# martenlienen/generative-turbulence

Hardware: AMD Instinct MI355X
Metric: U-Net fwd+bwd voxels/sec (DDPM training step, 192x64x48x4) (higher is better)
Workload: dtype bf16

## Files before the change

generative-turbulence_amd/csrc/tdx_conv3_ring.hip:

```cpp
#include "tdx_common.h"
#include "tdx_conv3.h"
#include "tdx_mfma.h"
#include <stdlib.h>
#include <algorithm>

#define RG_HY 10
#define RG_SZ 12
#define RG_SZ4 6
#define RG_WSLOTS 3
#define RG_WAVES 8
#define RG_STEPS 14
#ifndef RG_DEFAULT_LOADERS
#define RG_DEFAULT_LOADERS 1
#endif

struct RingArgs {
    const bf16* x1; const bf16* x2; int C1, C2;
    const bf16* wp; const float* bias; bf16* y;
    int B, X, Y, Z, Cout;
    int nbx, nby, nbz, ntn;
    double* gn_acc;
    bf16* d1; bf16* d2; int D1; const bf16* a1; const bf16* a2;
    const void* zeros;
    unsigned long long* stamps;
};

__device__ __forceinline__ void rg_dma_off(const void* sbase, unsigned voff, unsigned lds) {
    lds = __builtin_amdgcn_readfirstlane(lds);
    unsigned keep;
    asm volatile("s_mov_b32 %0, m0\n\ts_mov_b32 m0, %3\n\ts_nop 0\n\tglobal_load_lds_dwordx4 %1, %2\n\ts_mov_b32 m0, %0"
                 : "=&s"(keep) : "v"(voff), "s"(sbase), "s"(lds) : "memory");
}
#define RG_VMCNT(n) asm volatile("s_waitcnt vmcnt(%0)" ::"n"(n) : "memory")

#ifdef RG_STAMPS
#define RG_NSTAMP 64
#define RG_T()                                                                                        \
    do {                                                                                              \
        if (ord >= RG_STAMP_B0 && ord < RG_STAMP_B0 + 2) {                                            \
            const unsigned long long t_ = __builtin_amdgcn_s_memtime();                               \
            if (lane == 0 && nst < RG_NSTAMP) sStamp[wave * RG_NSTAMP + nst] = t_;                    \
            ++nst;                                                                                    \
        }                                                                                             \
    } while (0)
#else
#define RG_T() do { } while (0)
#endif

template <int BN>
__device__ __forceinline__ int rg_tile_addr(int v, int c) {
    if (BN == 64) return v * 128 + ((c ^ (v & 7)) << 4);
    return v * 64 + ((c ^ ((v >> 1) & 3)) << 4);
}

template <int NT, int LW = 0, bool Z4 = false>
struct RingShape {
    static constexpr int IW = LW ? LW : 8;
    static constexpr int BN = NT * 32;
    static constexpr int MT = 4 / NT;
    static constexpr int XP = Z4 ? MT : MT / 2;
    static constexpr int BX = 8 * XP;
    static constexpr int BZ = Z4 ? 4 : 8;
    static constexpr int HZ = BZ + 2;
    static constexpr int SZ = Z4 ? RG_SZ4 : RG_SZ;
    static constexpr int ENT = Z4 ? (BX + 2) / 2 * RG_HY * RG_SZ
                                  : (BX + 2) * RG_HY * SZ;
    static constexpr int APIECES = (ENT + 63) / 64;
    static constexpr int ABUF = APIECES * 1024;
    static constexpr int BPW = (APIECES + IW - 1) / IW;
    static constexpr int WPIECES = 28 * BN * 16 / 1024;
    static constexpr int WSLOT = WPIECES * 1024;
    static constexpr int WPW = (WPIECES + IW - 1) / IW;
    static constexpr int TILE = 32 * BN * 2;
    static constexpr int CH = BN / 8;
    static constexpr int VPI = 64 / CH;
    static constexpr int NST = MT * (32 / VPI);
    static constexpr size_t LDS = (size_t)2 * ABUF + (size_t)RG_WSLOTS * WSLOT + (size_t)RG_WAVES * TILE + 1024  +
                                  64  + BN * 4  + (size_t)RG_WAVES * BN * 2 * 4 ;
};

template <int NT, bool ZP, int LW, bool HF, bool Z4>
__global__ void __launch_bounds__(512 + 64 * LW, LW ? 3 : 2) conv3_ring_kernel(RingArgs A) {
    typedef RingShape<NT, LW, Z4> S;
    typedef H16<HF> H;
    typedef typename H::T HT;
    constexpr int BN = S::BN, MT = S::MT, XP = S::XP, BPW = S::BPW, WPW = S::WPW, CH = S::CH, VPI = S::VPI, NST = S::NST;
    static_assert(LW > 0 || BPW + WPW < RG_STEPS, "one DMA instruction per K step");
    extern __shared__ __attribute__((aligned(1024))) unsigned char smem[];
    unsigned char* sA = smem;
    unsigned char* sW = sA + 2 * S::ABUF;
    unsigned char* sT = sW + RG_WSLOTS * S::WSLOT;
    unsigned char* sD = sT + RG_WAVES * S::TILE;
    unsigned char* sZ = sD + 1024;
    float* sBias = reinterpret_cast<float*>(sZ + 64);
    float* sRed = sBias + BN;
    const unsigned lds0 = (unsigned)(size_t)(__attribute__((address_space(3))) const void*)smem;
    const unsigned ldsA = lds0, ldsW = lds0 + 2 * S::ABUF, ldsD = ldsW + RG_WSLOTS * S::WSLOT + RG_WAVES * S::TILE;

    const int tid = threadIdx.x, lane = tid & 63;
    const int wave = __builtin_amdgcn_readfirstlane(tid >> 6);
    const int r = lane & 31, hh = lane >> 5;
    const bool loader = LW > 0 && wave >= RG_WAVES;
    const int iw = LW ? wave - RG_WAVES : wave;
#ifdef RG_STAMPS
    unsigned long long* sStamp = reinterpret_cast<unsigned long long*>(NT == 2 ? sRed : sRed + RG_WAVES * BN * 2);
    int nst = 0;
#endif

    const int hw = blockIdx.x, xcd = hw & 7, slot = hw >> 3;
    const int ntile = slot % A.ntn, kx = slot / A.ntn, KX = (int)(gridDim.x >> 3) / A.ntn;
    const int nbricks = A.B * A.nbx * A.nby * A.nbz;
    const int lo = xcd * (nbricks >> 3) + min(xcd, nbricks & 7), hi = lo + (nbricks >> 3) + (xcd < (nbricks & 7) ? 1 : 0);
    const int nmine = hi - lo > kx ? (hi - lo - kx + KX - 1) / KX : 0;
    if (nmine == 0) return;
    const int n0 = ntile * BN;
    const int Cin = A.C1 + A.C2, nun = Cin >> 3;
    const int YZ = A.Y * A.Z, V = A.X * YZ;

    if (tid < BN) sBias[tid] = A.bias ? A.bias[n0 + tid] : 0.f;
    if (tid < 16) reinterpret_cast<unsigned*>(sZ)[tid] = 0u;
    lds_barrier();

    int hxyz[BPW];
#pragma unroll
    for (int i = 0; i < BPW; ++i) {
        const int pi = min(max(iw, 0) * BPW + i, S::APIECES - 1);
        const int e = min(pi * 64 + lane, S::ENT - 1);
        int hx, hy, hz;
        if (Z4) {
            const int xp = e / (RG_HY * RG_SZ), rem = e - xp * (RG_HY * RG_SZ), q = rem % RG_SZ;
            hy = rem / RG_SZ; hx = 2 * xp + q / RG_SZ4; hz = q % RG_SZ4;
        } else {
            hx = e / (RG_HY * S::SZ);
            const int rem = e - hx * (RG_HY * S::SZ);
            hy = rem / S::SZ; hz = min(rem - hy * S::SZ, S::HZ - 1);
        }
        hxyz[i] = hx | (hy << 8) | (hz << 16);
    }
    unsigned wlane[WPW];
#pragma unroll
    for (int j = 0; j < WPW; ++j) {
        const int pj = min(max(iw, 0) * WPW + j, S::WPIECES - 1);
        const int e = pj * 64 + lane;
        wlane[j] = (unsigned)((min(e / BN, 26) * A.Cout + (e % BN)) * 32);
    }

    const int ly = Z4 ? (r & 7) : (r & 3), lz = Z4 ? (r >> 3) : (r >> 2);
    int a_h[MT];
#pragma unroll
    for (int mt = 0; mt < MT; ++mt) {
        const int px = Z4 ? wave * XP + mt : wave * XP + mt / 2, py = Z4 ? ly : 4 * (mt % 2) + ly;
        const int hx = px + 1;
        a_h[mt] = Z4 ? ((hx >> 1) * (RG_HY * RG_SZ) + (py + 1) * RG_SZ + (hx & 1) * RG_SZ4 + (lz + 1)) * 16
                     : ((hx * RG_HY + (py + 1)) * S::SZ + (lz + 1)) * 16;
    }
    int xo[Z4 ? 2 : 1][RG_STEPS];
#pragma unroll
    for (int p = 0; p < RG_STEPS; ++p) {
        const int t = min(2 * p + hh, 26);
        const int dx = t / 9 - 1, dy = (t / 3) % 3 - 1, dz = t % 3 - 1;
        if (Z4) {
            const int step_odd = dx > 0 ? RG_HY * RG_SZ - RG_SZ4 : (dx < 0 ? -RG_SZ4 : 0);
            const int step_even = dx > 0 ? RG_SZ4 : (dx < 0 ? RG_SZ4 - RG_HY * RG_SZ : 0);
            xo[0][p] = (step_odd + dy * RG_SZ + dz) * 16;
            xo[Z4 ? 1 : 0][p] = (step_even + dy * RG_SZ + dz) * 16;
        } else {
            xo[0][p] = ((dx * RG_HY + dy) * S::SZ + dz) * 16;
        }
    }
    int b_off[NT];
#pragma unroll
    for (int nt = 0; nt < NT; ++nt) b_off[nt] = (hh * BN + nt * 32 + r) * 16;

    int vox[BPW];
    int vb_b = 0;
    auto brick_coords = [&](int ord, int& b, int& o0, int& o1, int& o2) {
        int id = lo + kx + KX * ord;
        const int bz = id % A.nbz; id /= A.nbz;
        const int by = id % A.nby; id /= A.nby;
        const int bx = id % A.nbx; id /= A.nbx;
        b = id; o0 = bx * S::BX; o1 = by * 8; o2 = bz * S::BZ;
    };
    auto plan_brick = [&](int ord) {
        int b, o0, o1, o2;
        brick_coords(min(ord, nmine - 1), b, o0, o1, o2);
        vb_b = b;
#pragma unroll
        for (int i = 0; i < BPW; ++i) {
            int s0 = o0 + (hxyz[i] & 0xff) - 1, s1 = o1 + ((hxyz[i] >> 8) & 0xff) - 1, s2 = o2 + ((hxyz[i] >> 16) & 0xff) - 1;
            bool ok = true;
            if (ZP) ok = s0 >= 0 && s0 < A.X && s1 >= 0 && s1 < A.Y && s2 >= 0 && s2 < A.Z;
            else { s0 = min(max(s0, 0), A.X - 1); s1 = min(max(s1, 0), A.Y - 1); s2 = min(max(s2, 0), A.Z - 1); }
            vox[i] = ok ? (s0 * A.Y + s1) * A.Z + s2 : -1;
        }
    };
    auto issue_brick_piece = [&](int c8, int buf, int i) {
        const int k0 = c8 << 3;
        const bf16* xs; int Cs, kk;
        if (k0 < A.C1) { xs = A.x1; Cs = A.C1; kk = k0; } else { xs = A.x2; Cs = A.C2; kk = k0 - A.C1; }
        const bf16* base = xs + ((int64_t)vb_b * V) * Cs + kk;
        const int pi = iw * BPW + i;
        const unsigned dst = pi < S::APIECES ? ldsA + buf * S::ABUF + pi * 1024 : ldsD;
        if (ZP) {
            const bf16* src = vox[i] >= 0 ? base + (int64_t)vox[i] * Cs : reinterpret_cast<const bf16*>(A.zeros);
            lds_dma16(src, dst);
        } else {
            rg_dma_off(base, (unsigned)(vox[i] * Cs) * 2u, dst);
        }
    };
    auto issue_weight_piece = [&](int c8, int wslot, int j) {
        const bf16* base = A.wp + ((int64_t)((c8 >> 1) * 27) * A.Cout + n0) * 16 + (c8 & 1) * 8;
        const int pj = iw * WPW + j;
        const unsigned dst = pj < S::WPIECES ? ldsW + wslot * S::WSLOT + pj * 1024 : ldsD;
        rg_dma_off(base, wlane[j], dst);
    };

    typedef __attribute__((ext_vector_type(2))) float f32x2;
    f32x2 p1[4], p2[4];
#pragma unroll
    for (int e = 0; e < 4; ++e) p1[e] = p2[e] = f32x2{0.f, 0.f};
    auto flush_stats = [&](int b) {
        float s1[8], s2[8];
#pragma unroll
        for (int e = 0; e < 4; ++e) { s1[2 * e] = p1[e].x; s1[2 * e + 1] = p1[e].y; s2[2 * e] = p2[e].x; s2[2 * e + 1] = p2[e].y; }
#pragma unroll
        for (int e = 0; e < 8; ++e) {
#pragma unroll
            for (int o = CH; o < 64; o <<= 1) { s1[e] += __shfl_xor(s1[e], o, 64); s2[e] += __shfl_xor(s2[e], o, 64); }
        }
        if (lane < CH) {
#pragma unroll
            for (int e = 0; e < 8; ++e) {
                sRed[(wave * BN + lane * 8 + e) * 2] = s1[e];
                sRed[(wave * BN + lane * 8 + e) * 2 + 1] = s2[e];
            }
        }
        lds_barrier();
        if (tid < BN * 2) {
            float t = 0.f;
#pragma unroll
            for (int w = 0; w < RG_WAVES; ++w) t += sRed[w * BN * 2 + tid];
            const int rep = blockIdx.x & (TDX_GN_REPLICAS - 1);
            atomicAdd(&A.gn_acc[(((size_t)rep * A.B + b) * A.Cout + n0) * 2 + tid], (double)t);
        }
        lds_barrier();
#pragma unroll
        for (int e = 0; e < 4; ++e) p1[e] = p2[e] = f32x2{0.f, 0.f};
    };

    int qs = 1, qb = 0, ws = 2 % nun, uw = 2;
    int u = 0;
    if (LW == 0 || loader) {
        plan_brick(0);
#pragma unroll
        for (int i = 0; i < BPW; ++i) issue_brick_piece(0, 0, i);
#pragma unroll
        for (int j = 0; j < WPW; ++j) issue_weight_piece(0, 0, j);
#pragma unroll
        for (int j = 0; j < WPW; ++j) issue_weight_piece(1 % nun, 1, j);
        if (qs == nun) { qs = 0; qb = 1; plan_brick(1); }
    }
    if (LW > 0 && loader) {
        for (int ord = 0; ord < nmine; ++ord) {
            for (int c8 = 0; c8 < nun; ++c8, ++u) {
                RG_VMCNT(WPW);
                lds_barrier();
#pragma unroll
                for (int i = 0; i < BPW; ++i) issue_brick_piece(qs, (u + 1) & 1, i);
#pragma unroll
                for (int j = 0; j < WPW; ++j) issue_weight_piece(ws, uw % RG_WSLOTS, j);
                ++uw;
                if (++ws == nun) ws = 0;
                if (++qs == nun) { qs = 0; ++qb; plan_brick(qb); }
            }
#ifndef RG_STAMPS
            if (!ZP && A.gn_acc != nullptr) {
                int b, nb = -1, t0, t1, t2;
                brick_coords(ord, b, t0, t1, t2);
                if (ord + 1 < nmine) brick_coords(ord + 1, nb, t0, t1, t2);
                if (nb != b) { lds_barrier(); lds_barrier(); }
            }
#endif
        }
        RG_VMCNT(0);
        return;
    }
    bool stores_behind = false;

    f32x16 acc[NT][MT];

    for (int ord = 0; ord < nmine; ++ord) {
        int b, o0, o1, o2;
        brick_coords(ord, b, o0, o1, o2);
#pragma unroll
        for (int nt = 0; nt < NT; ++nt)
#pragma unroll
            for (int j = 0; j < 4; ++j) {
                const float4 bv = *reinterpret_cast<const float4*>(sBias + nt * 32 + 8 * j + 4 * hh);
#pragma unroll
                for (int mt = 0; mt < MT; ++mt) {
                    acc[nt][mt][4 * j] = bv.x; acc[nt][mt][4 * j + 1] = bv.y; acc[nt][mt][4 * j + 2] = bv.z; acc[nt][mt][4 * j + 3] = bv.w;
                }
            }

        for (int c8 = 0; c8 < nun; ++c8, ++u) {
            RG_T();
            if (LW == 0) { if (stores_behind) RG_VMCNT(WPW + NST); else RG_VMCNT(WPW); }
            stores_behind = false;
            RG_T();
            lds_barrier();
            RG_T();

            const unsigned char* bufA = sA + (u & 1) * S::ABUF;
            const unsigned char* slotW = sW + (u % RG_WSLOTS) * S::WSLOT;
            const unsigned char* xa[MT];
#pragma unroll
            for (int mt = 0; mt < MT; ++mt) xa[mt] = bufA + a_h[mt];

            bf16x8 xf[3][MT], wf[3][NT];
            auto read_frags = [&](int p, int fb) {
#pragma unroll
                for (int mt = 0; mt < MT; ++mt) {
                    const unsigned char* src = xa[mt] + xo[Z4 ? (mt & 1) : 0][p];
                    if (p == RG_STEPS - 1) src = hh ? sZ : src;
                    xf[fb][mt] = *reinterpret_cast<const bf16x8*>(src);
                }
#pragma unroll
                for (int nt = 0; nt < NT; ++nt) wf[fb][nt] = *reinterpret_cast<const bf16x8*>(slotW + p * (2 * BN * 16) + b_off[nt]);
            };
            read_frags(0, 0);
            read_frags(1, 1);
            __builtin_amdgcn_sched_group_barrier(0x100, 2 * (MT + NT), 0);
#pragma unroll
            for (int p = 0; p < RG_STEPS; ++p) {
#if defined(RG_ABL) && (RG_ABL & 2)
                if (false)
#endif
                if (p + 2 < RG_STEPS) read_frags(p + 2, (p + 2) % 3);
#pragma unroll
                for (int nt = 0; nt < NT; ++nt)
#pragma unroll
                    for (int mt = 0; mt < MT; ++mt)
                        acc[nt][mt] = H::mfma(wf[p % 3][nt], xf[p % 3][mt], acc[nt][mt]);
                if (p + 2 < RG_STEPS) {
#pragma unroll
                    for (int k = 0; k < 4; ++k) {
                        __builtin_amdgcn_sched_group_barrier(0x008, 1, 0);
                        if (k < MT + NT) __builtin_amdgcn_sched_group_barrier(0x100, 1, 0);
                    }
                } else {
                    __builtin_amdgcn_sched_group_barrier(0x008, 4, 0);
                }
#if !defined(RG_ABL) || !(RG_ABL & 1)
                if (LW == 0 && p < BPW) issue_brick_piece(qs, (u + 1) & 1, p);
                if (LW == 0 && p >= BPW && p < BPW + WPW) issue_weight_piece(ws, uw % RG_WSLOTS, p - BPW);
#endif
                if (LW == 0 && p == BPW + WPW) {
                    ++uw;
                    if (++ws == nun) ws = 0;
                    if (++qs == nun) { qs = 0; ++qb; plan_brick(qb); }
                }
            }
        }

        RG_T();
        unsigned char* tile = sT + wave * S::TILE;
        const int last_b = b;
#pragma unroll
        for (int mt = 0; mt < MT; ++mt) {
            const int vw = ly * S::BZ + lz;
#pragma unroll
            for (int nt = 0; nt < NT; ++nt)
#pragma unroll
                for (int j = 0; j < 4; ++j) {
                    const int ch = nt * 32 + 8 * j + 4 * hh;
                    const unsigned lo2 = H::pack2(acc[nt][mt][4 * j], acc[nt][mt][4 * j + 1]);
                    const unsigned hi2 = H::pack2(acc[nt][mt][4 * j + 2], acc[nt][mt][4 * j + 3]);
                    *reinterpret_cast<uint2*>(tile + rg_tile_addr<BN>(vw, ch >> 3) + (ch & 7) * 2) = make_uint2(lo2, hi2);
                }
#pragma unroll
            for (int i = 0; i < 32 / VPI; ++i) {
                const int v = lane / CH + VPI * i, cidx = lane % CH;
                const int c0 = o0 + (Z4 ? wave * XP + mt : wave * XP + mt / 2);
                const int c1 = o1 + (Z4 ? (v >> 2) : 4 * (mt % 2) + (v >> 3)), c2 = o2 + (Z4 ? (v & 3) : (v & 7));
                uint4 val = *reinterpret_cast<const uint4*>(tile + rg_tile_addr<BN>(v, cidx));
                const int64_t ov = (int64_t)b * V + c0 * YZ + c1 * A.Z + c2;
                const int n = n0 + cidx * 8;
                if (ZP) {
                    const bool lo1 = n < A.D1;
                    bf16* dst = lo1 ? A.d1 + ov * A.D1 + n : A.d2 + ov * (A.Cout - A.D1) + (n - A.D1);
                    const bf16* asrc = lo1 ? (A.a1 ? A.a1 + ov * A.D1 + n : nullptr)
                                           : (A.a2 ? A.a2 + ov * (A.Cout - A.D1) + (n - A.D1) : nullptr);
                    if (asrc) {
                        Vec8<HT> va, vb;
                        va.load(reinterpret_cast<const HT*>(&val));
                        vb.load(reinterpret_cast<const HT*>(asrc));
#pragma unroll
                        for (int e = 0; e < 8; ++e) va.v[e] += vb.v[e];
                        va.store(reinterpret_cast<HT*>(dst));
                    } else {
                        *reinterpret_cast<uint4*>(dst) = val;
                    }
                } else {
                    *reinterpret_cast<uint4*>(A.y + ov * A.Cout + n) = val;
                    if (A.gn_acc != nullptr) {
                        const unsigned wds[4] = {val.x, val.y, val.z, val.w};
#pragma unroll
                        for (int e = 0; e < 4; ++e) {
                            const f32x2 lh = {H::lo(wds[e]), H::hi(wds[e])};
                            p1[e] += lh;
                            p2[e] = __builtin_elementwise_fma(lh, lh, p2[e]);
                        }
                    }
                }
            }
        }
        stores_behind = true;
        RG_T();
#ifndef RG_STAMPS
        if (!ZP && A.gn_acc != nullptr) {
            int nb = -1;
            if (ord + 1 < nmine) { int t0, t1, t2; brick_coords(ord + 1, nb, t0, t1, t2); }
            if (nb != last_b) flush_stats(last_b);
        }
#endif
    }
    if (LW == 0) RG_VMCNT(0);
#ifdef RG_STAMPS
    if (lane == 0 && A.stamps != nullptr) {
        unsigned long long* rec = A.stamps + ((size_t)blockIdx.x * RG_WAVES + wave) * (RG_NSTAMP + 1);
        rec[0] = nst;
        for (int i = 0; i < RG_NSTAMP; ++i) rec[1 + i] = sStamp[wave * RG_NSTAMP + i];
    }
#endif
}

static bool ring_z8_supported(int C1, int C2, int Cout, int B, int X, int Y, int Z, int mode);
static bool ring_z4_supported(int C1, int C2, int Cout, int B, int X, int Y, int Z, int mode) {
    const char* env = getenv("TDX_RING_Z4");
    if (env && atoi(env) == 0) return false;
    const int NT = Cout % 64 == 0 ? 2 : 1, bx = NT == 2 ? 16 : 32;
    if (X < bx || Y < 8 || Z < 4 || (X % bx) > 2 || (Y % 8) > 2 || (Z % 4) > 2) return false;
    const int ntn = Cout / (32 * NT);
    if (ntn > tdx_persistent_cus() / 8) return false;
    if ((int64_t)X * Y * Z * 1024 >= (1ll << 31)) return false;
    if (mode == 2) return true;
    if (NT == 1 && std::max(C1, C2) > 32) return false;
    const int64_t nb = (int64_t)B * (X / bx) * (Y / 8) * (Z / 4);
    return nb * ntn >= 192 && (C1 + C2) >= 64;
}
static int ring_brick_depth(int C1, int C2, int Cout, int B, int X, int Y, int Z) {
    const char* env = getenv("TDX_CONV3_RING");
    const int mode = env ? atoi(env) : 1;
    if (mode == 0 || !conv3_mfma_supported(C1, C2, Cout)) return 0;
    const char* z4 = getenv("TDX_RING_Z4");
    if (z4 && atoi(z4) == 2 && ring_z4_supported(C1, C2, Cout, B, X, Y, Z, 2)) return 4;
    if (ring_z8_supported(C1, C2, Cout, B, X, Y, Z, mode)) return 8;
    return ring_z4_supported(C1, C2, Cout, B, X, Y, Z, mode) ? 4 : 0;
}
int conv3_ring_depth(int C1, int C2, int N, int B, int X, int Y, int Z, bool data_gradient) {
    if (data_gradient && (tdx_scratch_ptr() == nullptr || tdx_scratch_bytes() < 16)) return 0;
    return ring_brick_depth(C1, C2, N, B, X, Y, Z);
}
static bool ring_z8_supported(int C1, int C2, int Cout, int B, int X, int Y, int Z, int mode) {
    const int NT = Cout % 64 == 0 ? 2 : 1, bx = NT == 2 ? 8 : 16;
    if (X < bx || Y < 8 || Z < 8 || (X % bx) > 2 || (Y % 8) > 2 || (Z % 8) > 2) return false;
    const char* rag = getenv("TDX_RING_RAGGED");
    if (rag && atoi(rag) == 0 && ((X % bx) || (Y % 8) || (Z % 8))) return false;
    const int ntn = Cout / (32 * NT);
    if (ntn > tdx_persistent_cus() / 8) return false;
    if ((int64_t)X * Y * Z * 1024 >= (1ll << 31)) return false;
    if (mode == 2) return true;
    if (NT == 1 && std::max(C1, C2) > 32) return false;
    const int64_t nb = (int64_t)B * (X / bx) * (Y / 8) * (Z / 8);
    const char* mi = getenv("TDX_RING_MIN_ITEMS");
    return nb * ntn >= (mi ? atoi(mi) : 3 * 256);
}

#ifdef RG_STAMPS
static unsigned long long* rg_stamp_buffer = nullptr;
#endif

template <int NT, bool ZP, int LW, bool HF, bool Z4 = false>
static int ring_go(const RingArgs& a, hipStream_t st) {
    size_t lds = RingShape<NT, LW, Z4>::LDS;
#ifdef RG_STAMPS
    if (NT == 1) lds += (size_t)RG_WAVES * RG_NSTAMP * 8;
#endif
    auto kern = conv3_ring_kernel<NT, ZP, LW, HF, Z4>;
    static bool attr_set = false;
    if (!attr_set) {
        hipError_t e = hipFuncSetAttribute((const void*)kern, hipFuncAttributeMaxDynamicSharedMemorySize, (int)lds);
        if (e != hipSuccess) return (int)e;
        attr_set = true;
    }
    const int px = tdx_persistent_cus() / 8, grid = 8 * (px - px % a.ntn);
    hipLaunchKernelGGL(kern, dim3(grid), dim3(512 + 64 * LW), lds, st, a);
    return tdx_launch_status();
}

int conv3_ring_launch(const Conv3Call& c, int depth) {
    if ((depth != 4 && depth != 8) || !tdx_is_h16(c.fmt)) return TDX_EINVAL;
    if (c.zero_pad && (tdx_scratch_ptr() == nullptr || tdx_scratch_bytes() < 16)) return TDX_EINVAL;
    const int X = c.X, Y = c.Y, Z = c.Z;
    const bool zero_pad = c.zero_pad, hf = c.hf();
    hipStream_t st = c.st;
    const int NT = c.N % 64 == 0 ? 2 : 1;
    const int bxr = (NT == 2 ? 8 : 16) * (depth == 4 ? 2 : 1);
    RingArgs a;
    a.x1 = (const bf16*)c.x1; a.x2 = (const bf16*)c.x2; a.C1 = c.C1; a.C2 = c.C2;
    a.wp = (const bf16*)c.wp; a.bias = c.bias; a.y = (bf16*)c.y;
    a.B = c.B; a.X = X; a.Y = Y; a.Z = Z; a.Cout = c.N;
    a.nbx = X / bxr; a.nby = Y / 8; a.nbz = Z / depth; a.ntn = c.N / (32 * NT);
    a.gn_acc = c.gn_acc;
    a.d1 = (bf16*)c.d1; a.d2 = (bf16*)c.d2; a.D1 = c.D1; a.a1 = (const bf16*)c.a1; a.a2 = (const bf16*)c.a2;
    a.zeros = tdx_scratch_ptr();
    a.stamps = nullptr;
#ifdef RG_STAMPS
    a.stamps = rg_stamp_buffer;
#endif
    const char* env = getenv("TDX_RING_LOADERS");
    const bool lw = env ? atoi(env) != 0 : RG_DEFAULT_LOADERS;
    int rc;
    if (depth == 4) {
#define RG_Z4(NTV) (hf ? (zero_pad ? ring_go<NTV, true, 4, true, true>(a, st) : ring_go<NTV, false, 4, true, true>(a, st)) \
                       : (zero_pad ? ring_go<NTV, true, 4, false, true>(a, st) : ring_go<NTV, false, 4, false, true>(a, st)))
        rc = NT == 2 ? RG_Z4(2) : RG_Z4(1);
#undef RG_Z4
    } else if (hf) {
        if (NT == 2) rc = zero_pad ? ring_go<2, true, 4, true>(a, st) : ring_go<2, false, 4, true>(a, st);
        else rc = zero_pad ? ring_go<1, true, 4, true>(a, st) : ring_go<1, false, 4, true>(a, st);
    } else if (NT == 2) {
        if (lw) rc = zero_pad ? ring_go<2, true, 4, false>(a, st) : ring_go<2, false, 4, false>(a, st);
        else rc = zero_pad ? ring_go<2, true, 0, false>(a, st) : ring_go<2, false, 0, false>(a, st);
    } else {
        if (lw) rc = zero_pad ? ring_go<1, true, 4, false>(a, st) : ring_go<1, false, 4, false>(a, st);
        else rc = zero_pad ? ring_go<1, true, 0, false>(a, st) : ring_go<1, false, 0, false>(a, st);
    }
    if (rc != TDX_OK || ((X % bxr) == 0 && (Y % 8) == 0 && (Z % depth) == 0)) return rc;
    const int beyond[3] = {X - X % bxr, Y - Y % 8, Z - Z % depth};
    Conv3Call rest = c;
    rest.slabs_beyond = beyond;
    return conv3_mfma_launch(rest);
}

extern "C" int tdx_conv3_uses_ring(int C1, int C2, int Cout, int B, int X, int Y, int Z) {
    return ring_brick_depth(C1, C2, Cout, B, X, Y, Z) != 0 ? 1 : 0;
}
extern "C" int tdx_conv3_ring_brick_depth(int C1, int C2, int Cout, int B, int X, int Y, int Z) {
    return ring_brick_depth(C1, C2, Cout, B, X, Y, Z);
}
```

Baseline: 166.7 million.

## Pair channel units to eliminate zero-padded 28th tap MFMA in ring conv

The 27 taps were padded to 28 (14 steps of 2 taps), so one MFMA step per channel unit multiplied against zeros. The K loop now handles channel-octet units in pairs: the even unit runs 13 steps and carries its leftover tap-27 fragment in registers, and the odd unit folds it into its first step, alongside shifted weight offsets. Across the two units this removes one of every 28 MFMA steps, at the cost of extra registers, more complex scheduling and a new requirement that C1 and C2 be multiples of 16.

```diff
diff --git a/generative-turbulence_amd/csrc/tdx_conv3_ring.hip b/generative-turbulence_amd/csrc/tdx_conv3_ring.hip
--- a/generative-turbulence_amd/csrc/tdx_conv3_ring.hip
+++ b/generative-turbulence_amd/csrc/tdx_conv3_ring.hip
@@ -3,6 +3,7 @@
 #include "tdx_mfma.h"
 #include <stdlib.h>
 #include <algorithm>
+#include <type_traits>
 
 #define RG_HY 10
 #define RG_SZ 12
@@ -10,6 +11,7 @@
 #define RG_WSLOTS 3
 #define RG_WAVES 8
 #define RG_STEPS 14
+#define RG_OWN 13
 #ifndef RG_DEFAULT_LOADERS
 #define RG_DEFAULT_LOADERS 1
 #endif
@@ -76,7 +78,7 @@
     static constexpr int VPI = 64 / CH;
     static constexpr int NST = MT * (32 / VPI);
     static constexpr size_t LDS = (size_t)2 * ABUF + (size_t)RG_WSLOTS * WSLOT + (size_t)RG_WAVES * TILE + 1024  +
-                                  64  + BN * 4  + (size_t)RG_WAVES * BN * 2 * 4 ;
+                                  BN * 4  + (size_t)RG_WAVES * BN * 2 * 4 ;
 };
 
 template <int NT, bool ZP, int LW, bool HF, bool Z4>
@@ -85,14 +87,13 @@
     typedef H16<HF> H;
     typedef typename H::T HT;
     constexpr int BN = S::BN, MT = S::MT, XP = S::XP, BPW = S::BPW, WPW = S::WPW, CH = S::CH, VPI = S::VPI, NST = S::NST;
-    static_assert(LW > 0 || BPW + WPW < RG_STEPS, "one DMA instruction per K step");
+    static_assert(LW > 0 || BPW + WPW < RG_OWN, "one DMA instruction per K step");
     extern __shared__ __attribute__((aligned(1024))) unsigned char smem[];
     unsigned char* sA = smem;
     unsigned char* sW = sA + 2 * S::ABUF;
     unsigned char* sT = sW + RG_WSLOTS * S::WSLOT;
     unsigned char* sD = sT + RG_WAVES * S::TILE;
-    unsigned char* sZ = sD + 1024;
-    float* sBias = reinterpret_cast<float*>(sZ + 64);
+    float* sBias = reinterpret_cast<float*>(sD + 1024);
     float* sRed = sBias + BN;
     const unsigned lds0 = (unsigned)(size_t)(__attribute__((address_space(3))) const void*)smem;
     const unsigned ldsA = lds0, ldsW = lds0 + 2 * S::ABUF, ldsD = ldsW + RG_WSLOTS * S::WSLOT + RG_WAVES * S::TILE;
@@ -118,7 +119,6 @@
     const int YZ = A.Y * A.Z, V = A.X * YZ;
 
     if (tid < BN) sBias[tid] = A.bias ? A.bias[n0 + tid] : 0.f;
-    if (tid < 16) reinterpret_cast<unsigned*>(sZ)[tid] = 0u;
     lds_barrier();
 
     int hxyz[BPW];
@@ -137,12 +137,13 @@
         }
         hxyz[i] = hx | (hy << 8) | (hz << 16);
     }
-    unsigned wlane[WPW];
+    unsigned wlane[WPW], wodd[WPW];
 #pragma unroll
     for (int j = 0; j < WPW; ++j) {
         const int pj = min(max(iw, 0) * WPW + j, S::WPIECES - 1);
         const int e = pj * 64 + lane;
         wlane[j] = (unsigned)((min(e / BN, 26) * A.Cout + (e % BN)) * 32);
+        wodd[j] = e / BN < 27 ? 16u : 0u;
     }
 
     const int ly = Z4 ? (r & 7) : (r & 3), lz = Z4 ? (r >> 3) : (r >> 2);
@@ -209,10 +210,10 @@
         }
     };
     auto issue_weight_piece = [&](int c8, int wslot, int j) {
-        const bf16* base = A.wp + ((int64_t)((c8 >> 1) * 27) * A.Cout + n0) * 16 + (c8 & 1) * 8;
+        const bf16* base = A.wp + ((int64_t)((c8 >> 1) * 27) * A.Cout + n0) * 16;
         const int pj = iw * WPW + j;
         const unsigned dst = pj < S::WPIECES ? ldsW + wslot * S::WSLOT + pj * 1024 : ldsD;
-        rg_dma_off(base, wlane[j], dst);
+        rg_dma_off(base, wlane[j] + ((c8 & 1) ? wodd[j] : 0u), dst);
     };
 
     typedef __attribute__((ext_vector_type(2))) float f32x2;
@@ -288,6 +289,7 @@
     bool stores_behind = false;
 
     f32x16 acc[NT][MT];
+    bf16x8 xcar[MT];
 
     for (int ord = 0; ord < nmine; ++ord) {
         int b, o0, o1, o2;
@@ -303,7 +305,9 @@
                 }
             }
 
-        for (int c8 = 0; c8 < nun; ++c8, ++u) {
+        auto unit = [&](auto odd_c) __attribute__((always_inline)) {
+            constexpr bool ODD = decltype(odd_c)::value;
+            constexpr int NQ = ODD ? RG_OWN + 1 : RG_OWN;
             RG_T();
             if (LW == 0) { if (stores_behind) RG_VMCNT(WPW + NST); else RG_VMCNT(WPW); }
             stores_behind = false;
@@ -318,49 +322,65 @@
             for (int mt = 0; mt < MT; ++mt) xa[mt] = bufA + a_h[mt];
 
             bf16x8 xf[3][MT], wf[3][NT];
-            auto read_frags = [&](int p, int fb) {
+            auto read_frags = [&](int q, int fb) {
+                const int p = ODD ? (q == 0 ? RG_STEPS - 1 : q - 1) : q;
 #pragma unroll
                 for (int mt = 0; mt < MT; ++mt) {
-                    const unsigned char* src = xa[mt] + xo[Z4 ? (mt & 1) : 0][p];
-                    if (p == RG_STEPS - 1) src = hh ? sZ : src;
-                    xf[fb][mt] = *reinterpret_cast<const bf16x8*>(src);
+                    if (ODD && q == 0) xf[fb][mt] = xcar[mt];
+                    else xf[fb][mt] = *reinterpret_cast<const bf16x8*>(xa[mt] + xo[Z4 ? (mt & 1) : 0][p]);
                 }
 #pragma unroll
                 for (int nt = 0; nt < NT; ++nt) wf[fb][nt] = *reinterpret_cast<const bf16x8*>(slotW + p * (2 * BN * 16) + b_off[nt]);
             };
+            if (ODD && hh == 0) {
+#pragma unroll
+                for (int mt = 0; mt < MT; ++mt)
+                    xcar[mt] = *reinterpret_cast<const bf16x8*>(xa[mt] + xo[Z4 ? (mt & 1) : 0][RG_STEPS - 1]);
+            }
             read_frags(0, 0);
             read_frags(1, 1);
             __builtin_amdgcn_sched_group_barrier(0x100, 2 * (MT + NT), 0);
 #pragma unroll
-            for (int p = 0; p < RG_STEPS; ++p) {
+            for (int q = 0; q < NQ; ++q) {
+                const int nrd = q + 2 < NQ ? MT + NT : (!ODD && q + 2 == NQ ? MT : 0);
 #if defined(RG_ABL) && (RG_ABL & 2)
                 if (false)
 #endif
-                if (p + 2 < RG_STEPS) read_frags(p + 2, (p + 2) % 3);
+                if (q + 2 < NQ) read_frags(q + 2, (q + 2) % 3);
+                if (!ODD && q + 2 == NQ) {
+#pragma unroll
+                    for (int mt = 0; mt < MT; ++mt)
+                        xcar[mt] = *reinterpret_cast<const bf16x8*>(xa[mt] + xo[Z4 ? (mt & 1) : 0][RG_STEPS - 1]);
+                }
 #pragma unroll
                 for (int nt = 0; nt < NT; ++nt)
 #pragma unroll
                     for (int mt = 0; mt < MT; ++mt)
-                        acc[nt][mt] = H::mfma(wf[p % 3][nt], xf[p % 3][mt], acc[nt][mt]);
-                if (p + 2 < RG_STEPS) {
+                        acc[nt][mt] = H::mfma(wf[q % 3][nt], xf[q % 3][mt], acc[nt][mt]);
+                if (nrd) {
 #pragma unroll
                     for (int k = 0; k < 4; ++k) {
                         __builtin_amdgcn_sched_group_barrier(0x008, 1, 0);
-                        if (k < MT + NT) __builtin_amdgcn_sched_group_barrier(0x100, 1, 0);
+                        if (k < nrd) __builtin_amdgcn_sched_group_barrier(0x100, 1, 0);
                     }
                 } else {
                     __builtin_amdgcn_sched_group_barrier(0x008, 4, 0);
                 }
 #if !defined(RG_ABL) || !(RG_ABL & 1)
-                if (LW == 0 && p < BPW) issue_brick_piece(qs, (u + 1) & 1, p);
-                if (LW == 0 && p >= BPW && p < BPW + WPW) issue_weight_piece(ws, uw % RG_WSLOTS, p - BPW);
-#endif
-                if (LW == 0 && p == BPW + WPW) {
+                if (LW == 0 && q < BPW) issue_brick_piece(qs, (u + 1) & 1, q);
+                if (LW == 0 && q >= BPW && q < BPW + WPW) issue_weight_piece(ws, uw % RG_WSLOTS, q - BPW);
+#endif
+                if (LW == 0 && q == BPW + WPW) {
                     ++uw;
                     if (++ws == nun) ws = 0;
                     if (++qs == nun) { qs = 0; ++qb; plan_brick(qb); }
                 }
             }
+            ++u;
+        };
+        for (int c8 = 0; c8 < nun; c8 += 2) {
+            unit(std::false_type{});
+            unit(std::true_type{});
         }
 
         RG_T();
@@ -453,6 +473,7 @@
     const char* env = getenv("TDX_CONV3_RING");
     const int mode = env ? atoi(env) : 1;
     if (mode == 0 || !conv3_mfma_supported(C1, C2, Cout)) return 0;
+    if ((C1 % 16) != 0 || (C2 % 16) != 0) return 0;
     const char* z4 = getenv("TDX_RING_Z4");
     if (z4 && atoi(z4) == 2 && ring_z4_supported(C1, C2, Cout, B, X, Y, Z, 2)) return 4;
     if (ring_z8_supported(C1, C2, Cout, B, X, Y, Z, mode)) return 8;
@@ -501,6 +522,7 @@
 
 int conv3_ring_launch(const Conv3Call& c, int depth) {
     if ((depth != 4 && depth != 8) || !tdx_is_h16(c.fmt)) return TDX_EINVAL;
+    if (c.C1 <= 0 || (c.C1 % 16) != 0 || (c.C2 % 16) != 0) return TDX_EINVAL;
     if (c.zero_pad && (tdx_scratch_ptr() == nullptr || tdx_scratch_bytes() < 16)) return TDX_EINVAL;
     const int X = c.X, Y = c.Y, Z = c.Z;
     const bool zero_pad = c.zero_pad, hf = c.hf();
```

Measured after the change: 166.7 million (median of 2 runs). Within noise of the previous version (+0.0%).
